# Tomiinek/Multilingual_Text_to_Speech

Measured on NVIDIA H100. Metric: mel-frames/sec (train fwd+bwd), higher is better.
Workload: dtype bf16

## Files before the change

### multilingual_text_to_speech_b200/csrc/decoder_persist_tc.cu

```cuda
#include <cuda.h>
#include <cuda_bf16.h>
#include "decoder_internal.cuh"
#include "tc_ptx.cuh"

namespace b200tts {

int tc_make_map3_bf16(void* map, const void* base, int d0, int d1, int d2, size_t stride1, size_t stride2, int b0, int b1, int b2);

namespace {

constexpr int NCW = 8;
constexpr int CT = 32 * NCW;
constexpr int PT = CT + 128;
constexpr int UNITS = 16;
constexpr int ROWS = 4 * UNITS;
constexpr int BT = 32;
constexpr int KB = 64;
constexpr int WTILE = ROWS * KB * 2;
constexpr int ATILE = BT * KB * 2;

struct TcLoopArgs {
    int B, T, D, K, Kp, RB, NBH;
    int nkb, nkb_h;
    int ch_h, n_h, ch_c, n_c, slot_kb;
    int alias_sum;
    int use_btab;
    const float* W; int ldw; int wcol_h, wcol_c;
    __nv_bfloat16* actb;
    float* actf; int ldf; int hcol;
    float* gates;
    float* cstate;
    const uint8_t* mask_h; const uint8_t* mask_c;
    int kind, training; float rate_h, rate_c;
    int L, M, A, KC;
    const float* Wq; float* qpart; float* qsave;
    const __nv_bfloat16* WcB;
    const __nv_bfloat16* memTf; int MT;
    const float* bias; const float* v;
    const uint4* memFf; int M16;
    const int* lengths;
    float* cum; float* align; long long align_bstride;
    unsigned* barrier; int* abort_flag;
    long long* prof;
    long long* prof2;
};

__device__ __forceinline__ uint32_t smem_u32(const void* p) { return (uint32_t)__cvta_generic_to_shared(p); }
__device__ __forceinline__ void mbar_init(uint64_t* bar, uint32_t count) {
    asm volatile("mbarrier.init.shared::cta.b64 [%0], %1;" ::"r"(smem_u32(bar)), "r"(count));
}
__device__ __forceinline__ void mbar_expect_tx(uint64_t* bar, uint32_t bytes) {
    asm volatile("mbarrier.arrive.expect_tx.shared::cta.b64 _, [%0], %1;" ::"r"(smem_u32(bar)), "r"(bytes) : "memory");
}
__device__ __forceinline__ void mbar_wait(uint64_t* bar, uint32_t parity) {
    const uint32_t addr = smem_u32(bar);
    const long long t0 = clock64();
    for (;;) {
        uint32_t done;
        asm volatile(
            "{\n\t.reg .pred p;\n\t"
            "mbarrier.try_wait.parity.shared::cta.b64 p, [%1], %2;\n\t"
            "selp.u32 %0, 1, 0, p;\n\t}"
            : "=r"(done)
            : "r"(addr), "r"(parity)
            : "memory");
        if (done) return;
        if (clock64() - t0 > 4000000000ll) __trap();
    }
}
__device__ __forceinline__ void tma_load_3d(void* smem, const CUtensorMap* map, uint64_t* bar, int c0, int c1, int c2) {
    asm volatile(
        "cp.async.bulk.tensor.3d.shared::cluster.global.mbarrier::complete_tx::bytes [%0], [%1, {%3, %4, %5}], [%2];"
        ::"r"(smem_u32(smem)), "l"(reinterpret_cast<uint64_t>(map)), "r"(smem_u32(bar)), "r"(c0), "r"(c1), "r"(c2)
        : "memory");
}
__device__ __forceinline__ void proxy_fence_global() { asm volatile("fence.proxy.async.global;" ::: "memory"); }
__device__ __forceinline__ void proxy_fence_shared() { asm volatile("fence.proxy.async.shared::cta;" ::: "memory"); }
__device__ __forceinline__ bool elect_one() {
    uint32_t pred;
    asm volatile("{\n\t.reg .pred P;\n\telect.sync _|P, 0xffffffff;\n\tselp.u32 %0, 1, 0, P;\n\t}" : "=r"(pred));
    return pred != 0;
}
__device__ __forceinline__ void l2_prefetch(const void* p) { asm volatile("prefetch.global.L2 [%0];" ::"l"(p)); }
__device__ __forceinline__ void cluster_arrive() { asm volatile("barrier.cluster.arrive.release.aligned;" ::: "memory"); }
__device__ __forceinline__ void cluster_wait() { asm volatile("barrier.cluster.wait.acquire.aligned;" ::: "memory"); }
__device__ __forceinline__ void st_peer_f32(const float* local_smem, uint32_t peer_rank, float v) {
    uint32_t ra;
    asm volatile("mapa.shared::cluster.u32 %0, %1, %2;" : "=r"(ra) : "r"(smem_u32(local_smem)), "r"(peer_rank));
    asm volatile("st.shared::cluster.f32 [%0], %1;" ::"r"(ra), "f"(v) : "memory");
}
__device__ __forceinline__ void st_async_peer_f32(const float* local_smem, const uint64_t* local_bar, uint32_t peer_rank, float v) {
    uint32_t ra, rb;
    asm volatile("mapa.shared::cluster.u32 %0, %1, %2;" : "=r"(ra) : "r"(smem_u32(local_smem)), "r"(peer_rank));
    asm volatile("mapa.shared::cluster.u32 %0, %1, %2;" : "=r"(rb) : "r"(smem_u32(local_bar)), "r"(peer_rank));
    asm volatile("st.async.shared::cluster.mbarrier::complete_tx::bytes.b32 [%0], %1, [%2];" ::"r"(ra), "r"(__float_as_uint(v)), "r"(rb) : "memory");
}
__device__ __forceinline__ void csync() { asm volatile("bar.sync 1, %0;" ::"n"(CT) : "memory"); }

__device__ __forceinline__ void ldmatrix_x4(uint32_t& r0, uint32_t& r1, uint32_t& r2, uint32_t& r3, const void* p) {
    const uint32_t addr = (uint32_t)__cvta_generic_to_shared(p);
    asm volatile("ldmatrix.sync.aligned.m8n8.x4.shared.b16 {%0,%1,%2,%3}, [%4];\n" : "=r"(r0), "=r"(r1), "=r"(r2), "=r"(r3) : "r"(addr));
}
__device__ __forceinline__ void mma_bf16(float (&c)[4], const uint32_t (&a)[4], uint32_t b0, uint32_t b1) {
    asm volatile("mma.sync.aligned.m16n8k16.row.col.f32.bf16.bf16.f32 {%0,%1,%2,%3}, {%4,%5,%6,%7}, {%8,%9}, {%0,%1,%2,%3};\n"
                 : "+f"(c[0]), "+f"(c[1]), "+f"(c[2]), "+f"(c[3])
                 : "r"(a[0]), "r"(a[1]), "r"(a[2]), "r"(a[3]), "r"(b0), "r"(b1));
}
__device__ __forceinline__ unsigned ld_acquire(const unsigned* p) {
    unsigned v;
    asm volatile("ld.acquire.gpu.global.u32 %0, [%1];\n" : "=r"(v) : "l"(p) : "memory");
    return v;
}
__device__ __forceinline__ uint32_t pack2(float lo, float hi) {
    __nv_bfloat162 v = __floats2bfloat162_rn(lo, hi);
    return *reinterpret_cast<uint32_t*>(&v);
}
__device__ __forceinline__ float tanh_fast(float x) {
    float y;
    asm("tanh.approx.f32 %0, %1;" : "=f"(y) : "f"(x));
    return y;
}

__device__ __forceinline__ float sigmoid_fast(float x) { return __fdividef(1.f, 1.f + __expf(-x)); }
__device__ __forceinline__ float tanh_exp(float x) { return 2.f * __fdividef(1.f, 1.f + __expf(-2.f * x)) - 1.f; }

__device__ __forceinline__ float cblock_max(float v, float* scratch) {
    const int lane = threadIdx.x & 31, warp = threadIdx.x >> 5;
    v = warp_max(v);
    csync();
    if (lane == 0) scratch[warp] = v;
    csync();
    float t = scratch[lane & (NCW - 1)];
#pragma unroll
    for (int o = NCW / 2; o > 0; o >>= 1) t = fmaxf(t, __shfl_xor_sync(0xffffffffu, t, o));
    return t;
}
__device__ __forceinline__ float cblock_sum(float v, float* scratch) {
    const int lane = threadIdx.x & 31, warp = threadIdx.x >> 5;
    v = warp_sum(v);
    csync();
    if (lane == 0) scratch[warp] = v;
    csync();
    float t = scratch[lane & (NCW - 1)];
#pragma unroll
    for (int o = NCW / 2; o > 0; o >>= 1) t += __shfl_xor_sync(0xffffffffu, t, o);
    return t;
}

struct NoOverlap { __device__ __forceinline__ void operator()() const {} };
template <typename Overlap = NoOverlap>
__device__ __forceinline__ bool grid_barrier(unsigned* counter, unsigned& target, unsigned nblocks, int* abort_flag, int* s_ok, Overlap overlap = Overlap()) {
    __syncthreads();
    if (threadIdx.x == 0) {
        target += nblocks;
        proxy_fence_global();
        asm volatile("red.release.gpu.global.add.u32 [%0], 1;" ::"l"(counter) : "memory");
    }
    overlap();
    if (threadIdx.x == 0) {
        int ok = 1;
        const long long t0 = clock64();
        unsigned polls = 0;
        for (;;) {
            unsigned v;
            asm volatile("ld.relaxed.gpu.global.u32 %0, [%1];" : "=r"(v) : "l"(counter) : "memory");
            if (v >= target) break;
            if ((++polls & 255u) == 0 && (clock64() - t0 > 4000000000ll || *reinterpret_cast<volatile int*>(abort_flag))) {
                ok = 0; *abort_flag = 1; break;
            }
        }
        asm volatile("fence.acquire.gpu;" ::: "memory");
        *s_ok = ok;
    }
    __syncthreads();
    return *s_ok != 0;
}

template <bool ATT, bool ALIAS>
__global__ void __launch_bounds__(PT, 1) lstm_loop_tc_kernel(const __grid_constant__ CUtensorMap tmH, const __grid_constant__ CUtensorMap tmC,
                                                             const TcLoopArgs p) {
    extern __shared__ __align__(1024) unsigned char smem_raw0[];
    unsigned char* smem_raw = reinterpret_cast<unsigned char*>((reinterpret_cast<uintptr_t>(smem_raw0) + 1023) & ~(uintptr_t)1023);
    __shared__ uint64_t full_bar, full2_bar, accum_bar, xchg_bar;
    __shared__ int s_ok;

    const int tid = threadIdx.x, lane = tid & 31;
    const int warp = __shfl_sync(0xffffffffu, tid >> 5, 0);
    const int cta = blockIdx.x;
    const int rb = cta % p.RB, bh = cta / p.RB;
    const int u0 = rb * UNITS, b0 = bh * BT;
    const int Kp = p.Kp, D = p.D, B = p.B;
    const unsigned nblocks = gridDim.x;
    unsigned* const bar_counter = p.barrier;
    const bool compute = warp < NCW;
    const bool is_mma = warp >= NCW;

    size_t off = 0;
    unsigned char* sW = smem_raw + off; off += (size_t)p.nkb * WTILE;
    unsigned char* ring = smem_raw + off;
    {
        const size_t ring_b = (size_t)p.slot_kb * ATILE, sum_b = (size_t)BT * (ROWS + 1) * 4;
        off += ALIAS ? (ring_b > sum_b ? ring_b : sum_b) : ring_b;
    }
    float* s_sum = ALIAS ? reinterpret_cast<float*>(ring) : reinterpret_cast<float*>(smem_raw + off);
    off += ALIAS ? 0 : (size_t)BT * (ROWS + 1) * 4;
    float* s_hs = reinterpret_cast<float*>(smem_raw + off); off += ATT ? (size_t)UNITS * (BT + 4) * 4 : 0;
    __nv_bfloat16* sWcB = reinterpret_cast<__nv_bfloat16*>(smem_raw + off); off += ATT ? (size_t)(p.A / 2) * 40 * 2 : 0;
    float* scratch = reinterpret_cast<float*>(smem_raw + off);

    for (int idx = tid; idx < ROWS * p.nkb * KB; idx += PT) {
        const int r = idx / (p.nkb * KB), k = idx % (p.nkb * KB);
        const int g = r / UNITS, u = r % UNITS;
        float w = 0.f;
        if (k < p.K && u0 + u < D) w = p.W[(size_t)(g * D + u0 + u) * p.ldw + (k < D ? p.wcol_h + k : p.wcol_c + (k - D))];
        const int kb = k / KB, kc = k % KB, chunk = kc >> 3, e = kc & 7;
        *reinterpret_cast<__nv_bfloat16*>(sW + (size_t)kb * WTILE + r * 128 + ((chunk ^ (r & 7)) << 4) + e * 2) = __float2bfloat16_rn(w);
    }
    if (ATT) {
        for (int idx = tid; idx < (p.A / 2) * 40; idx += PT) sWcB[idx] = p.WcB[(size_t)(cta & 1) * (p.A / 2) * 40 + idx];
    }
    if (tid == 0) {
        mbar_init(&full_bar, 1); mbar_init(&full2_bar, 1); mbar_init(&xchg_bar, 1);
        mbar_init(&accum_bar, 128);
        asm volatile("fence.mbarrier_init.release.cluster;" ::: "memory");
    }
    proxy_fence_shared();
    __syncthreads();
    if (ATT) { cluster_arrive(); cluster_wait(); }

    uint32_t mma_it = 0;
    long long rp[4] = {0, 0, 0, 0};
    float acc[16];
    auto mma_part = [&](int step, int part, bool signal_accum) {
        const long long t0 = clock64();
        long long t1 = t0;
        const int n = part ? p.n_h : (ALIAS ? p.n_c : 1), ch = part ? p.ch_h : p.ch_c;
        if (!ATT) {
            if (warp == NCW) {
                proxy_fence_global();
                if (elect_one()) {
                    for (int j = 0; j < n; ++j) {
                        uint64_t* fb = j ? &full2_bar : &full_bar;
                        mbar_expect_tx(fb, (uint32_t)ch * ATILE);
                        tma_load_3d(ring + (size_t)j * ch * ATILE, &tmH, fb, 0, step * B + b0, j * ch);
                    }
                }
                __syncwarp();
            }
            for (int j = 0; j < n; ++j) {
                mbar_wait(j ? &full2_bar : &full_bar, mma_it & 1);
                if (j == 0) t1 = clock64();
                tcx::wgmma_fence();
                for (int c = 0; c < ch; ++c) {
                    const uint64_t adesc = tcx::make_sw128_desc(smem_u32(sW + (size_t)(j * ch + c) * WTILE));
                    const uint64_t bdesc = tcx::make_sw128_desc(smem_u32(ring + (size_t)(j * ch + c) * ATILE));
#pragma unroll
                    for (int k = 0; k < KB / 16; ++k) tcx::wgmma_m64n32<0, 0>(acc, adesc + 2 * k, bdesc + 2 * k, (j | c | k) != 0);
                }
                tcx::wgmma_commit();
            }
            ++mma_it;
            tcx::wgmma_wait<0>();
            tcx::wgmma_fence_acc(acc);
        } else {
            for (int j = 0; j < n; ++j) {
                if (warp == NCW) {
                    if (j == 0) proxy_fence_global();
                    if (elect_one()) {
                        if (ALIAS) proxy_fence_shared();
                        mbar_expect_tx(&full_bar, (uint32_t)ch * ATILE);
                        tma_load_3d(ring, part ? &tmH : &tmC, &full_bar, 0, step * B + b0, part ? j * ch : p.nkb_h + j * ch);
                    }
                    __syncwarp();
                }
                mbar_wait(&full_bar, mma_it & 1);
                ++mma_it;
                if (j == 0) t1 = clock64();
                const int kb0 = part ? j * ch : p.nkb_h + j * ch;
                tcx::wgmma_fence();
                for (int c = 0; c < ch; ++c) {
                    const uint64_t adesc = tcx::make_sw128_desc(smem_u32(sW + (size_t)(kb0 + c) * WTILE));
                    const uint64_t bdesc = tcx::make_sw128_desc(smem_u32(ring + (size_t)c * ATILE));
#pragma unroll
                    for (int k = 0; k < KB / 16; ++k)
                        tcx::wgmma_m64n32<0, 0>(acc, adesc + 2 * k, bdesc + 2 * k, (part == 1 && j == 0 && c == 0 && k == 0) ? 0u : 1u);
                }
                tcx::wgmma_commit();
                tcx::wgmma_wait<0>();
                tcx::wgmma_fence_acc(acc);
                tcx::wg_sync(NCW / 4);
            }
        }
        if (signal_accum) {
            const int row = 16 * (warp - NCW) + (lane >> 2), col = 2 * (lane & 3);
#pragma unroll
            for (int r = 0; r < 16; ++r) s_sum[(8 * (r >> 2) + col + (r & 1)) * (ROWS + 1) + row + 8 * ((r >> 1) & 1)] = acc[r];
            tcx::mbar_arrive(&accum_bar);
        }
        rp[2 * part] += t1 - t0; rp[2 * part + 1] += clock64() - t1;
    };

    uint32_t wqh[2][2] = {{0u, 0u}, {0u, 0u}}, wql[2][2] = {{0u, 0u}, {0u, 0u}};
    if (ATT && compute) {
        const int g = lane >> 2, tq = lane & 3;
#pragma unroll
        for (int j = 0; j < 2; ++j)
#pragma unroll
            for (int r2 = 0; r2 < 2; ++r2) {
                const int a = (2 * warp + j) * 8 + g, u = u0 + 2 * tq + 8 * r2;
                const float x0 = (a < p.A && u < D) ? p.Wq[(size_t)a * D + u] : 0.f, x1 = (a < p.A && u + 1 < D) ? p.Wq[(size_t)a * D + u + 1] : 0.f;
                const __nv_bfloat16 h0 = __float2bfloat16_rn(x0), h1 = __float2bfloat16_rn(x1);
                __nv_bfloat162 hp2; hp2.x = h0; hp2.y = h1;
                wqh[j][r2] = *reinterpret_cast<uint32_t*>(&hp2);
                wql[j][r2] = pack2(x0 - __bfloat162float(h0), x1 - __bfloat162float(h1));
            }
    }
    const float inv_h = 1.f / (1.f - p.rate_h), inv_c = 1.f / (1.f - p.rate_c);
    unsigned target = 0;
    long long prof_acc[8] = {0, 0, 0, 0, 0, 0, 0, 0};
    long long prof_t = clock64();
#define PROF_MARK(slot)                                                      \
    do {                                                                     \
        if (p.prof && tid == 0) { const long long now = clock64(); prof_acc[slot] += now - prof_t; prof_t = now; } \
    } while (0)

    if (is_mma) mma_part(0, 1, !ATT || p.nkb_h == p.nkb);

    float pre[2][6];
    uint8_t pm[2][2];
    auto prefetch = [&](int step, bool state) {
#pragma unroll
        for (int e2 = 0; e2 < 2; ++e2) {
            const int idx = tid + e2 * CT;
            const int bl = idx / UNITS, uu = idx % UNITS, b = b0 + bl, u = u0 + uu;
            pm[e2][0] = 1; pm[e2][1] = 1;
#pragma unroll
            for (int j = 0; j < 4; ++j) pre[e2][j] = 0.f;
            if (state) { pre[e2][4] = 0.f; pre[e2][5] = 0.f; }
            if (b < B && u < D) {
                const size_t g0 = ((size_t)step * B + b) * 4 * D + u, mi = ((size_t)step * B + b) * D + u;
                pre[e2][0] = p.gates[g0]; pre[e2][1] = p.gates[g0 + D]; pre[e2][2] = p.gates[g0 + 2 * D]; pre[e2][3] = p.gates[g0 + 3 * D];
                if (state) {
                    pre[e2][4] = p.cstate[mi];
                    pre[e2][5] = p.actf[((size_t)step * B + b) * p.ldf + p.hcol + u];
                }
                if (p.training && p.mask_h) pm[e2][0] = p.mask_h[mi];
                if (p.training && p.mask_c) pm[e2][1] = p.mask_c[mi];
            }
        }
    };
    auto prefetch_l2 = [&](int step) {
        if (step >= p.T) return;
#pragma unroll
        for (int e2 = 0; e2 < 2; ++e2) {
            const int idx = tid + e2 * CT;
            const int bl = idx / UNITS, uu = idx % UNITS, b = b0 + bl, u = u0 + uu;
            if (b < B && u < D && (uu & 7) == 0) {
                const size_t g0 = ((size_t)step * B + b) * 4 * D + u, mi = ((size_t)step * B + b) * D + u;
                l2_prefetch(p.gates + g0); l2_prefetch(p.gates + g0 + D); l2_prefetch(p.gates + g0 + 2 * D); l2_prefetch(p.gates + g0 + 3 * D);
                if (uu == 0 && p.training && p.mask_h) l2_prefetch(p.mask_h + mi);
                if (uu == 0 && p.training && p.mask_c) l2_prefetch(p.mask_c + mi);
            }
        }
    };
    if (compute) { prefetch_l2(0); prefetch(0, true); prefetch_l2(1); }

    int att_len = 0;
    if (ATT && (cta >> 1) < B) { const int l0 = p.lengths[cta >> 1]; att_len = l0 < 0 ? 0 : (l0 > p.L ? p.L : l0); }
    bool alive = true;
    for (int i = 0; i < p.T && alive; ++i) {
        if (ATT && p.nkb_h < p.nkb && is_mma) mma_part(i, 0, true);
        if (compute) {
            mbar_wait(&accum_bar, i & 1);
            PROF_MARK(0);
#pragma unroll
            for (int e2 = 0; e2 < 2; ++e2) {
                const int idx = tid + e2 * CT;
                const int bl = idx / UNITS, uu = idx % UNITS, b = b0 + bl, u = u0 + uu;
                float hs = 0.f;
                if (b < B && u < D) {
                    const size_t g0 = ((size_t)i * B + b) * 4 * D + u;
                    const float zi = pre[e2][0] + s_sum[bl * (ROWS + 1) + uu];
                    const float zf = pre[e2][1] + s_sum[bl * (ROWS + 1) + UNITS + uu];
                    const float zg = pre[e2][2] + s_sum[bl * (ROWS + 1) + 2 * UNITS + uu];
                    const float zo = pre[e2][3] + s_sum[bl * (ROWS + 1) + 3 * UNITS + uu];
                    const float gi = sigmoid_fast(zi), gf = sigmoid_fast(zf), gg = tanh_exp(zg), go = sigmoid_fast(zo);
                    const size_t bu = (size_t)b * D + u;
                    const float cp = pre[e2][4];
                    float cn = gf * cp + gi * gg;
                    float hn = go * tanh_exp(cn);
                    p.gates[g0] = gi; p.gates[g0 + D] = gf; p.gates[g0 + 2 * D] = gg; p.gates[g0 + 3 * D] = go;
                    if (p.kind == B200TTS_CELL_ZONEOUT) {
                        const float hp = pre[e2][5];
                        if (p.training) {
                            float dh = hn - hp, dc = cn - cp;
                            if (p.mask_h) dh = dh * (float)pm[e2][0] * inv_h;
                            if (p.mask_c) dc = dc * (float)pm[e2][1] * inv_c;
                            hn = (1.f - p.rate_h) * dh + hp;
                            cn = (1.f - p.rate_c) * dc + cp;
                        } else {
                            hn = p.rate_h * hp + (1.f - p.rate_h) * hn;
                            cn = p.rate_c * cp + (1.f - p.rate_c) * cn;
                        }
                    } else if (p.training && p.mask_h) {
                        hn = hn * (float)pm[e2][0] * inv_h;
                    }
                    p.cstate[(size_t)(i + 1) * B * D + bu] = cn;
                    p.actf[((size_t)(i + 1) * B + b) * p.ldf + p.hcol + u] = hn;
                    p.actb[((size_t)(i + 1) * B + b) * Kp + u] = __float2bfloat16_rn(hn);
                    hs = hn;
                    pre[e2][4] = cn; pre[e2][5] = hn;
                }
                if (ATT) s_hs[uu * (BT + 4) + bl] = hs;
            }
            if (ATT) {
                csync();
                {
                    const int g = lane >> 2, tq = lane & 3;
                    uint32_t ah[2][4], al[2][4];
#pragma unroll
                    for (int mt = 0; mt < 2; ++mt)
#pragma unroll
                        for (int r4 = 0; r4 < 4; ++r4) {
                            const int bl = mt * 16 + g + 8 * (r4 & 1), k = 2 * tq + 8 * (r4 >> 1);
                            const float x0 = s_hs[k * (BT + 4) + bl], x1 = s_hs[(k + 1) * (BT + 4) + bl];
                            const __nv_bfloat16 h0 = __float2bfloat16_rn(x0), h1 = __float2bfloat16_rn(x1);
                            __nv_bfloat162 hp2; hp2.x = h0; hp2.y = h1;
                            ah[mt][r4] = *reinterpret_cast<uint32_t*>(&hp2);
                            al[mt][r4] = pack2(x0 - __bfloat162float(h0), x1 - __bfloat162float(h1));
                        }
#pragma unroll
                    for (int mt = 0; mt < 2; ++mt)
#pragma unroll
                        for (int j = 0; j < 2; ++j) {
                            float acc[4] = {0.f, 0.f, 0.f, 0.f};
                            mma_bf16(acc, ah[mt], wqh[j][0], wqh[j][1]);
                            mma_bf16(acc, al[mt], wqh[j][0], wqh[j][1]);
                            mma_bf16(acc, ah[mt], wql[j][0], wql[j][1]);
                            const int a = (2 * warp + j) * 8 + 2 * tq;
                            const int bA = b0 + mt * 16 + g, bB = bA + 8;
                            if (bA < B) *reinterpret_cast<float2*>(p.qpart + ((size_t)rb * B + bA) * p.A + a) = make_float2(acc[0], acc[1]);
                            if (bB < B) *reinterpret_cast<float2*>(p.qpart + ((size_t)rb * B + bB) * p.A + a) = make_float2(acc[2], acc[3]);
                        }
                }
            }
        }
        PROF_MARK(1);
        if (ALIAS) proxy_fence_shared();
        if (!grid_barrier(bar_counter, target, nblocks, p.abort_flag, &s_ok)) { alive = false; break; }
        PROF_MARK(2);

        if (i + 1 < p.T) {
            if (is_mma) mma_part(i + 1, 1, !ATT || p.nkb_h == p.nkb);
            if (compute) { prefetch_l2(i + 2); if (!ATT) prefetch(i + 1, false); }
        }

        if (ATT) {
            const int pc = cta >> 1, hf = cta & 1;
            if (compute && pc < B) {
                const int b = pc, L = p.L, A = p.A, AH = p.A / 2, M = p.M, half = (p.KC - 1) / 2, L16 = p.MT * 16;
                float* qb = scratch;
                float* vv = qb + AH;
                float* bias_s = vv + AH;
                float* cum_s = bias_s + AH;
                float* e = cum_s + L16;
                float* eq = e + L16;
                float* epart = eq + 2 * L16;
                float* red = epart + 2 * L16;
                float* cred = red + 64;
                uint32_t* Ph = reinterpret_cast<uint32_t*>(cred + 16 * AH);
                uint32_t* Pl = Ph + (L16 + 48);
                uint2* btab = reinterpret_cast<uint2*>(Pl + (L16 + 48));
                const int len = att_len;
                const int mtiles = (len + 15) / 16, ktiles = mtiles;
                if (i == 0) {
                    for (int a2 = tid; a2 < AH; a2 += CT) { vv[a2] = p.v[hf * AH + a2]; bias_s[a2] = p.bias[hf * AH + a2]; }
                    for (int l = tid; l < L16; l += CT) cum_s[l] = l < L ? p.cum[(size_t)b * L + l] : 0.f;
                    csync();
                }
                constexpr int KTMAX = 12;
                const int mt_lo = hf * ((p.M16 + 1) / 2), mt_hi = min(p.M16, mt_lo + (p.M16 + 1) / 2);
                uint4 nraw[2];
                uint4 av[KTMAX];
                {
                    const int a4 = tid & 15, sl = tid >> 4;
                    const int per = (p.RB + 15) / 16, r0 = sl * per, r1 = min(p.RB, r0 + per);
                    float4 qv[4];
#pragma unroll
                    for (int j = 0; j < 4; ++j)
                        qv[j] = (r0 + j < r1) ? __ldcg(reinterpret_cast<const float4*>(p.qpart + ((size_t)(r0 + j) * B + b) * A + hf * AH) + a4)
                                              : make_float4(0.f, 0.f, 0.f, 0.f);
                    if (warp < 2 * mtiles) {
                        const uint4* mf = reinterpret_cast<const uint4*>(p.memTf + (((size_t)b * p.MT + (warp >> 1)) * 32 + lane) * 64) + hf * 4 + (warp & 1) * 2;
                        nraw[0] = __ldg(mf); nraw[1] = __ldg(mf + 1);
                    }
                    if (mt_lo + warp < mt_hi) {
                        const uint4* fr = p.memFf + (((size_t)b * p.M16 + mt_lo + warp) * p.MT) * 32 + lane;
#pragma unroll
                        for (int j = 0; j < KTMAX; ++j)
                            if (j < ktiles) av[j] = __ldg(fr + (size_t)j * 32);
                    }
                    for (int x = tid; x < L16 + 48; x += CT) {
                        float c0 = 0.f, c1 = 0.f;
                        const int la = x - half, lb = x + 1 - half;
                        if (la >= 0 && la < L) c0 = cum_s[la];
                        if (lb >= 0 && lb < L) c1 = cum_s[lb];
                        const __nv_bfloat16 h0 = __float2bfloat16_rn(c0), h1 = __float2bfloat16_rn(c1);
                        __nv_bfloat162 hp2; hp2.x = h0; hp2.y = h1;
                        Ph[x] = *reinterpret_cast<uint32_t*>(&hp2);
                        Pl[x] = pack2(c0 - __bfloat162float(h0), c1 - __bfloat162float(h1));
                    }
                    float4 qs = make_float4(0.f, 0.f, 0.f, 0.f);
#pragma unroll
                    for (int j = 0; j < 4; ++j) { qs.x += qv[j].x; qs.y += qv[j].y; qs.z += qv[j].z; qs.w += qv[j].w; }
                    for (int r = r0 + 4; r < r1; r += 4) {
#pragma unroll
                        for (int j = 0; j < 4; ++j)
                            if (r + j < r1) {
                                const float4 v4 = __ldcg(reinterpret_cast<const float4*>(p.qpart + ((size_t)(r + j) * B + b) * A + hf * AH) + a4);
                                qs.x += v4.x; qs.y += v4.y; qs.z += v4.z; qs.w += v4.w;
                            }
                    }
                    *reinterpret_cast<float4*>(cred + sl * AH + a4 * 4) = qs;
                    csync();
                    for (int a2 = tid; a2 < AH; a2 += CT) {
                        float q = 0.f;
#pragma unroll
                        for (int sl2 = 0; sl2 < 16; ++sl2) q += cred[sl2 * AH + a2];
                        p.qsave[((size_t)i * B + b) * A + hf * AH + a2] = q;
                        qb[a2] = q + bias_s[a2];
                    }
                }
                csync();
                PROF_MARK(3);
                {
                    const int g = lane >> 2, tq = lane & 3;
                    for (int job = warp; job < 2 * mtiles; job += NCW) {
                        const int mt = job >> 1, qh = job & 1, l0 = mt * 16;
                        const uint4 raw[2] = {nraw[0], nraw[1]};
                        if (job + NCW < 2 * mtiles) {
                            const int nj = job + NCW;
                            const uint4* mf = reinterpret_cast<const uint4*>(p.memTf + (((size_t)b * p.MT + (nj >> 1)) * 32 + lane) * 64) + hf * 4 + (nj & 1) * 2;
                            nraw[0] = __ldg(mf); nraw[1] = __ldg(mf + 1);
                        }
                        float sacc[4][4];
#pragma unroll
                        for (int nt = 0; nt < 4; ++nt)
#pragma unroll
                            for (int e4 = 0; e4 < 4; ++e4) sacc[nt][e4] = 0.f;
#pragma unroll
                        for (int ks = 0; ks < 2; ++ks) {
                            const int x = l0 + ks * 16 + g + 2 * tq;
                            const uint32_t ah[4] = {Ph[x], Ph[x + 8], Ph[x + 8], Ph[x + 16]};
                            const uint32_t al[4] = {Pl[x], Pl[x + 8], Pl[x + 8], Pl[x + 16]};
#pragma unroll
                            for (int np = 0; np < 2; ++np) {
                                uint32_t bfr[4];
                                ldmatrix_x4(bfr[0], bfr[1], bfr[2], bfr[3],
                                            sWcB + (size_t)((qh * 2 + np) * 16 + (lane & 7) + ((lane >> 4) << 3)) * 40 + ks * 16 + ((lane >> 3) & 1) * 8);
                                mma_bf16(sacc[2 * np], ah, bfr[0], bfr[1]);
                                mma_bf16(sacc[2 * np], al, bfr[0], bfr[1]);
                                mma_bf16(sacc[2 * np + 1], ah, bfr[2], bfr[3]);
                                mma_bf16(sacc[2 * np + 1], al, bfr[2], bfr[3]);
                            }
                        }
                        float e0 = 0.f, e1 = 0.f;
#pragma unroll
                        for (int c4 = 0; c4 < 2; ++c4) {
                            const uint32_t words[4] = {raw[c4].x, raw[c4].y, raw[c4].z, raw[c4].w};
#pragma unroll
                            for (int h2 = 0; h2 < 2; ++h2) {
                                const int nt = 2 * c4 + h2, a0 = (qh * 4 + nt) * 8 + 2 * tq;
                                const float2 m01 = __bfloat1622float2(*reinterpret_cast<const __nv_bfloat162*>(&words[2 * h2]));
                                const float2 m23 = __bfloat1622float2(*reinterpret_cast<const __nv_bfloat162*>(&words[2 * h2 + 1]));
                                e0 = fmaf(vv[a0], tanh_fast(sacc[nt][0] + qb[a0] + m01.x), e0);
                                e0 = fmaf(vv[a0 + 1], tanh_fast(sacc[nt][1] + qb[a0 + 1] + m01.y), e0);
                                e1 = fmaf(vv[a0], tanh_fast(sacc[nt][2] + qb[a0] + m23.x), e1);
                                e1 = fmaf(vv[a0 + 1], tanh_fast(sacc[nt][3] + qb[a0 + 1] + m23.y), e1);
                            }
                        }
                        e0 += __shfl_xor_sync(0xffffffffu, e0, 1); e0 += __shfl_xor_sync(0xffffffffu, e0, 2);
                        e1 += __shfl_xor_sync(0xffffffffu, e1, 1); e1 += __shfl_xor_sync(0xffffffffu, e1, 2);
                        if (tq == 0) { eq[qh * L16 + l0 + g] = e0; eq[qh * L16 + l0 + g + 8] = e1; }
                    }
                }
                csync();
                if (tid == 0) mbar_expect_tx(&xchg_bar, (uint32_t)L16 * 4);
                for (int l = tid; l < L16; l += CT) {
                    const float v = l < mtiles * 16 ? eq[l] + eq[L16 + l] : 0.f;
                    epart[hf * L16 + l] = v;
                    st_async_peer_f32(epart + hf * L16 + l, &xchg_bar, (uint32_t)(hf ^ 1), v);
                }
                csync();
                mbar_wait(&xchg_bar, i & 1);
                PROF_MARK(4);
                float mx = -INFINITY;
                for (int l = tid; l < len; l += CT) { const float ev = epart[l] + epart[L16 + l]; e[l] = ev; mx = fmaxf(mx, ev); }
                mx = cblock_max(mx, red);
                float sum = 0.f;
                for (int l = tid; l < len; l += CT) { const float ex = expf(e[l] - mx); e[l] = ex; sum += ex; }
                sum = cblock_sum(sum, red + 32);
                float* cum_next = p.cum + ((size_t)(i + 1) * B + b) * L;
                const float inv_sum = 1.f / sum;
                for (int l = tid; l < L16; l += CT) {
                    const float w = l < len ? e[l] * inv_sum : 0.f;
                    e[l] = w;
                    if (l < L) {
                        const float cn = cum_s[l] + w;
                        cum_s[l] = cn;
                        if (hf == 0) p.align[(size_t)b * p.align_bstride + (size_t)i * L + l] = w;
                        else cum_next[l] = cn;
                    }
                }
                csync();
                if (p.use_btab) {
                    for (int idx = tid; idx < ktiles * 32; idx += CT) {
                        const int kt = idx >> 5, gg = (idx >> 2) & 7, tt = idx & 3;
                        uint2 f = make_uint2(0u, 0u);
                        if (gg < 2) {
                            const float* wl = e + kt * 16 + 2 * tt;
                            const float w0 = wl[0], w1 = wl[1], w2 = wl[8], w3 = wl[9];
                            const float h0 = __bfloat162float(__float2bfloat16_rn(w0)), h1 = __bfloat162float(__float2bfloat16_rn(w1));
                            const float h2 = __bfloat162float(__float2bfloat16_rn(w2)), h3 = __bfloat162float(__float2bfloat16_rn(w3));
                            f = gg == 0 ? make_uint2(pack2(h0, h1), pack2(h2, h3)) : make_uint2(pack2(w0 - h0, w1 - h1), pack2(w2 - h2, w3 - h3));
                        }
                        btab[idx] = f;
                    }
                    csync();
                }
                PROF_MARK(5);
                {
                    const int g = lane >> 2, tq = lane & 3;
                    uint32_t bfr[KTMAX][2];
                    auto build_b = [&](int kt0) {
                        if (p.use_btab) {
#pragma unroll
                            for (int j = 0; j < KTMAX; ++j) {
                                bfr[j][0] = 0u; bfr[j][1] = 0u;
                                if (kt0 + j < ktiles) { const uint2 f = btab[(kt0 + j) * 32 + lane]; bfr[j][0] = f.x; bfr[j][1] = f.y; }
                            }
                            return;
                        }
#pragma unroll
                        for (int j = 0; j < KTMAX; ++j) {
                            bfr[j][0] = 0u; bfr[j][1] = 0u;
                            if (kt0 + j < ktiles) {
                                const float* wl = e + (kt0 + j) * 16 + 2 * tq;
                                const float w0 = wl[0], w1 = wl[1], w2 = wl[8], w3 = wl[9];
                                const float h0 = __bfloat162float(__float2bfloat16_rn(w0)), h1 = __bfloat162float(__float2bfloat16_rn(w1));
                                const float h2 = __bfloat162float(__float2bfloat16_rn(w2)), h3 = __bfloat162float(__float2bfloat16_rn(w3));
                                const float s0 = g == 0 ? h0 : (g == 1 ? w0 - h0 : 0.f), s1 = g == 0 ? h1 : (g == 1 ? w1 - h1 : 0.f);
                                const float s2 = g == 0 ? h2 : (g == 1 ? w2 - h2 : 0.f), s3 = g == 0 ? h3 : (g == 1 ? w3 - h3 : 0.f);
                                bfr[j][0] = pack2(s0, s1); bfr[j][1] = pack2(s2, s3);
                            }
                        }
                    };
                    const bool single = ktiles <= KTMAX;
                    if (single) build_b(0);
                    for (int mt = mt_lo + warp; mt < mt_hi; mt += NCW) {
                        float dacc[4] = {0.f, 0.f, 0.f, 0.f}, dacc2[4] = {0.f, 0.f, 0.f, 0.f};
                        for (int kt0 = 0; kt0 < ktiles; kt0 += KTMAX) {
                            if (kt0 > 0 || mt != mt_lo + warp) {
                                const uint4* fr = p.memFf + (((size_t)b * p.M16 + mt) * p.MT) * 32 + lane;
#pragma unroll
                                for (int j = 0; j < KTMAX; ++j)
                                    if (kt0 + j < ktiles) av[j] = __ldg(fr + (size_t)(kt0 + j) * 32);
                            }
                            if (!single) build_b(kt0);
#pragma unroll
                            for (int j = 0; j < KTMAX; j += 2) {
                                if (kt0 + j < ktiles) {
                                    const uint32_t af[4] = {av[j].x, av[j].y, av[j].z, av[j].w};
                                    mma_bf16(dacc, af, bfr[j][0], bfr[j][1]);
                                }
                                if (kt0 + j + 1 < ktiles) {
                                    const uint32_t af[4] = {av[j + 1].x, av[j + 1].y, av[j + 1].z, av[j + 1].w};
                                    mma_bf16(dacc2, af, bfr[j + 1][0], bfr[j + 1][1]);
                                }
                            }
                        }
                        if (tq == 0) {
                            const int m0 = mt * 16 + g;
                            const float c0 = (dacc[0] + dacc2[0]) + (dacc[1] + dacc2[1]), c1 = (dacc[2] + dacc2[2]) + (dacc[3] + dacc2[3]);
                            if (m0 < M) {
                                p.actf[((size_t)(i + 1) * B + b) * p.ldf + m0] = c0;
                                p.actb[((size_t)(i + 1) * B + b) * Kp + D + m0] = __float2bfloat16_rn(c0);
                            }
                            if (m0 + 8 < M) {
                                p.actf[((size_t)(i + 1) * B + b) * p.ldf + m0 + 8] = c1;
                                p.actb[((size_t)(i + 1) * B + b) * Kp + D + m0 + 8] = __float2bfloat16_rn(c1);
                            }
                        }
                    }
                }
            }
            PROF_MARK(6);
            if (!grid_barrier(bar_counter, target, nblocks, p.abort_flag, &s_ok, [&]() { if (compute && i + 1 < p.T) prefetch(i + 1, false); })) {
                alive = false; break;
            }
            PROF_MARK(7);
        }
    }
    if (p.prof && tid == 0)
        for (int k = 0; k < 8; ++k) p.prof[(size_t)cta * 8 + k] = prof_acc[k];
#undef PROF_MARK
    if (p.prof2 && warp == NCW && lane == 0)
        for (int k = 0; k < 4; ++k) p.prof2[(size_t)cta * 8 + k] = rp[k];
}

size_t tc_loop_smem_bytes(int nkb, int slot_kb, int A, bool att, int L, bool alias = false) {
    const size_t ring_b = (size_t)slot_kb * ATILE, sum_b = (size_t)BT * (ROWS + 1) * 4;
    size_t b = 1024 + (size_t)nkb * WTILE + (alias ? (ring_b > sum_b ? ring_b : sum_b) : ring_b + sum_b);
    if (att) {
        const int L16 = (L + 15) / 16 * 16;
        b += (size_t)UNITS * (BT + 4) * 4 + (size_t)(A / 2) * 40 * 2;
        b += ((size_t)3 * (A / 2) + 6 * L16 + 64 + 16 * (A / 2) + 2 * (L16 + 48)) * 4;
    }
    return b;
}
constexpr size_t SMEM_LIMIT = 227 * 1024 - 1088;

int pick_slot(int nkb, int A, bool att, int L, int want, bool alias = false) {
    int kb = want;
    while (kb >= 1 && tc_loop_smem_bytes(nkb, kb, A, att, L, alias) > SMEM_LIMIT) --kb;
    return kb;
}
int largest_divisor_le(int n, int cap) {
    for (int d = cap < n ? cap : n; d >= 1; --d)
        if (n % d == 0) return d;
    return 1;
}

}

TcPersistGeom tc_persist_geom(const b200tts_decoder_shape& s) {
    TcPersistGeom g{};
    g.nkb_att = (s.D + s.M + KB - 1) / KB;
    g.nkb_gen = (s.D + KB - 1) / KB;
    g.nkb_h = s.D / KB;
    g.Kp_att = g.nkb_att * KB;
    g.Kp_gen = g.nkb_gen * KB;
    const int nkb_c = g.nkb_att - g.nkb_h;
    g.alias_att = 0;
    g.slot_att = pick_slot(g.nkb_att, s.A, true, s.L, g.nkb_h);
    if (g.slot_att < nkb_c) {
        g.alias_att = 1;
        g.slot_att = pick_slot(g.nkb_att, s.A, true, s.L, g.nkb_h, true);
    }
    g.ch_c_att = g.slot_att >= 1 ? largest_divisor_le(nkb_c, g.slot_att) : 0;
    g.n_c_att = g.ch_c_att >= 1 ? nkb_c / g.ch_c_att : 0;
    g.ch_h_att = g.slot_att >= 1 ? largest_divisor_le(g.nkb_h, g.slot_att) : 0;
    g.slot_gen = pick_slot(g.nkb_gen, s.A, false, 0, g.nkb_gen);
    g.ch_h_gen = g.slot_gen >= 1 ? largest_divisor_le(g.nkb_gen, g.slot_gen) : 0;
    if (g.slot_gen >= g.nkb_gen && g.nkb_gen % 2 == 0) g.ch_h_gen = g.nkb_gen / 2;
    return g;
}

bool tc_persist_supported(const b200tts_decoder_shape& s) {
    if (s.D % KB != 0 || s.D % UNITS != 0) return false;
    const int RB = s.D / UNITS, NBH = (s.B + BT - 1) / BT;
    if (RB * NBH > NUM_SMS || s.B > RB * NBH) return false;
    if (s.K > 32 || s.A != 128) return false;
    const TcPersistGeom g = tc_persist_geom(s);
    return g.ch_c_att >= 1 && g.ch_c_att <= 256 && g.slot_att >= g.ch_c_att && g.ch_h_att >= 1 && g.ch_h_gen >= 1 && g.slot_att >= 2 &&
           g.slot_gen >= g.nkb_gen;
}

static int launch_tc_loop(bool att, const TcLoopArgs& a, const CUtensorMap& tmH, const CUtensorMap& tmC, size_t smem, cudaStream_t st) {
    void* fn = att ? (a.alias_sum ? (void*)lstm_loop_tc_kernel<true, true> : (void*)lstm_loop_tc_kernel<true, false>) : (void*)lstm_loop_tc_kernel<false, false>;
    B200_CUDA(cudaFuncSetAttribute(fn, cudaFuncAttributeMaxDynamicSharedMemorySize, (int)smem));
    const int grid = a.RB * a.NBH;
    TcLoopArgs args = a;
    CUtensorMap mapH = tmH, mapC = tmC;
    void* params[] = {&mapH, &mapC, &args};
    cudaLaunchConfig_t cfg{};
    cfg.gridDim = dim3(grid); cfg.blockDim = dim3(PT); cfg.dynamicSmemBytes = smem; cfg.stream = st;
    cudaLaunchAttribute attrs[2];
    attrs[0].id = cudaLaunchAttributeCooperative;
    attrs[0].val.cooperative = 1;
    cfg.attrs = attrs; cfg.numAttrs = 1;
    if (att) {
        B200_REQUIRE(grid % 2 == 0 && grid / 2 >= a.B, "wgmma attention loop: %d CTAs cannot form %d pairs", grid, a.B);
        attrs[1].id = cudaLaunchAttributeClusterDimension;
        attrs[1].val.clusterDim.x = 2; attrs[1].val.clusterDim.y = 1; attrs[1].val.clusterDim.z = 1;
        cfg.numAttrs = 2;
        int nclusters = 0;
        B200_CUDA(cudaOccupancyMaxActiveClusters(&nclusters, fn, &cfg));
        B200_REQUIRE(nclusters * 2 >= grid, "wgmma attention loop: only %d CTA pairs can be co-resident, %d needed", nclusters, grid / 2);
    } else {
        int per_sm = 0, dev = 0, sms = 0;
        B200_CUDA(cudaOccupancyMaxActiveBlocksPerMultiprocessor(&per_sm, fn, PT, smem));
        B200_CUDA(cudaGetDevice(&dev));
        B200_CUDA(cudaDeviceGetAttribute(&sms, cudaDevAttrMultiProcessorCount, dev));
        B200_REQUIRE(per_sm * sms >= grid, "wgmma persistent loop: %d CTAs cannot be co-resident (%d per SM x %d SMs)", grid, per_sm, sms);
    }
    KernelTimer kt(att ? "lstm_loop_tc_kernel<att>" : "lstm_loop_tc_kernel<gen>", st);
    B200_CUDA(cudaLaunchKernelExC(&cfg, fn, params));
    B200_LAUNCH_CHECK();
    return B200TTS_OK;
}

int tc_persist_att_loop(const b200tts_decoder_shape& s, const b200tts_decoder_params& w, const b200tts_decoder_inputs& in,
                        const DecoderLayout& fl, float* ws, unsigned char* pws, float* align, cudaStream_t st) {
    const PersistLayout l = persist_layout(s);
    const TcPersistGeom g = tc_persist_geom(s);
    const int B = s.B, T = s.T, D = s.D, M = s.M, MD = M + D;
    __nv_bfloat16* aib = reinterpret_cast<__nv_bfloat16*>(pws + l.aib);
    unsigned* barrier = reinterpret_cast<unsigned*>(pws + l.barrier);
    B200_CUDA(cudaMemsetAsync(aib, 0, (size_t)(g.Kp_att != MD ? (size_t)(T + 1) : 1) * B * g.Kp_att * 2, st));
    B200_CUDA(cudaMemsetAsync(barrier, 0, 256, st));
    CUtensorMap tmH, tmC;
    B200_TRY(tc_make_map3_bf16(&tmH, aib, KB, (T + 1) * B, g.nkb_att, (size_t)g.Kp_att * 2, 128, KB, BT, g.ch_h_att));
    B200_TRY(tc_make_map3_bf16(&tmC, aib, KB, (T + 1) * B, g.nkb_att, (size_t)g.Kp_att * 2, 128, KB, BT, g.ch_c_att));
    TcLoopArgs a{};
    a.B = B; a.T = T; a.D = D; a.K = MD; a.Kp = g.Kp_att; a.RB = D / UNITS; a.NBH = (B + BT - 1) / BT;
    a.nkb = g.nkb_att; a.nkb_h = g.nkb_h; a.ch_h = g.ch_h_att; a.n_h = g.nkb_h / g.ch_h_att; a.ch_c = g.ch_c_att; a.n_c = g.n_c_att;
    a.alias_sum = g.alias_att;
    a.slot_kb = g.ch_h_att > g.ch_c_att ? g.ch_h_att : g.ch_c_att;
    a.W = ws + fl.wcat_att; a.ldw = MD; a.wcol_h = M; a.wcol_c = 0;
    a.actb = aib; a.actf = ws + fl.ai; a.ldf = MD; a.hcol = M;
    a.gates = ws + fl.ga; a.cstate = ws + fl.ca;
    a.mask_h = in.mask_att_h; a.mask_c = in.mask_att_c; a.kind = s.cell_kind; a.training = s.training; a.rate_h = s.rate_h; a.rate_c = s.rate_c;
    a.L = s.L; a.M = M; a.A = s.A; a.KC = s.K;
    a.Wq = w.attn_query; a.qpart = ws + fl.qpart; a.qsave = ws + fl.q;
    a.WcB = reinterpret_cast<const __nv_bfloat16*>(pws + l.wcb);
    a.memTf = reinterpret_cast<const __nv_bfloat16*>(pws + l.memTf); a.MT = l.MT;
    a.bias = w.attn_bias; a.v = w.attn_energy;
    a.memFf = reinterpret_cast<const uint4*>(pws + l.memFf); a.M16 = l.M16;
    a.lengths = in.text_lengths; a.cum = ws + fl.cum;
    a.align = align; a.align_bstride = (long long)T * s.L;
    a.barrier = barrier; a.abort_flag = reinterpret_cast<int*>(barrier + 32);
    a.prof = reinterpret_cast<long long*>(pws + l.barrier + 256);
    a.prof2 = a.prof + 2 * NUM_SMS * 8;
    size_t smem = tc_loop_smem_bytes(g.nkb_att, a.slot_kb, s.A, true, s.L, g.alias_att != 0);
    const size_t tab = (size_t)l.MT * 32 * 8;
    a.use_btab = smem + tab <= SMEM_LIMIT ? 1 : 0;
    if (a.use_btab) smem += tab;
    return launch_tc_loop(true, a, tmH, tmC, smem, st);
}

int tc_persist_gen_loop(const b200tts_decoder_shape& s, const b200tts_decoder_params& w, const b200tts_decoder_inputs& in,
                        const DecoderLayout& fl, float* ws, unsigned char* pws, cudaStream_t st) {
    const PersistLayout l = persist_layout(s);
    const TcPersistGeom g = tc_persist_geom(s);
    const int B = s.B, T = s.T, D = s.D;
    __nv_bfloat16* hgb = reinterpret_cast<__nv_bfloat16*>(pws + l.hgb);
    unsigned* barrier = reinterpret_cast<unsigned*>(pws + l.barrier);
    B200_CUDA(cudaMemsetAsync(hgb, 0, (size_t)(g.Kp_gen != D ? (size_t)(T + 1) : 1) * B * g.Kp_gen * 2, st));
    B200_CUDA(cudaMemsetAsync(barrier, 0, 256, st));
    CUtensorMap tmH;
    B200_TRY(tc_make_map3_bf16(&tmH, hgb, KB, (T + 1) * B, g.nkb_gen, (size_t)g.Kp_gen * 2, 128, KB, BT, g.ch_h_gen));
    TcLoopArgs a{};
    a.B = B; a.T = T; a.D = D; a.K = D; a.Kp = g.Kp_gen; a.RB = D / UNITS; a.NBH = (B + BT - 1) / BT;
    a.nkb = g.nkb_gen; a.nkb_h = g.nkb_gen; a.ch_h = g.ch_h_gen; a.n_h = g.nkb_gen / g.ch_h_gen; a.ch_c = 0; a.n_c = 0; a.alias_sum = 0; a.use_btab = 0; a.slot_kb = g.nkb_gen;
    a.W = w.gen_w_hh; a.ldw = D; a.wcol_h = 0; a.wcol_c = 0;
    a.actb = hgb; a.actf = ws + fl.hg; a.ldf = D; a.hcol = 0;
    a.gates = ws + fl.gg; a.cstate = ws + fl.cg;
    a.mask_h = in.mask_gen_h; a.mask_c = in.mask_gen_c; a.kind = s.cell_kind; a.training = s.training; a.rate_h = s.rate_h; a.rate_c = s.rate_c;
    a.barrier = barrier; a.abort_flag = reinterpret_cast<int*>(barrier + 32);
    a.prof = reinterpret_cast<long long*>(pws + l.barrier + 256) + NUM_SMS * 8;
    a.prof2 = a.prof + 2 * NUM_SMS * 8;
    return launch_tc_loop(false, a, tmH, tmH, tc_loop_smem_bytes(g.nkb_gen, a.slot_kb, s.A, false, 0), st);
}

}
```

Before: 677,700.

## Specialize MMA and compute warps with setmaxnreg register rebalancing

Splits the persistent LSTM kernel into two warp roles with separate control flow. The MMA producer warps run their own loop, mirroring the grid barrier with paired __syncthreads and exit early, after lowering their register budget with setmaxnreg.dec. The compute warps raise their budget with setmaxnreg.inc so the gate and attention code has more registers and spills less. The trap path moves into a noinline function, and the profiling accumulators move to shared memory in the attention variant to save registers. The main risk is barrier-count mismatch between the two roles, which could deadlock or mis-synchronise.

New measurement: 743,600, median of 6. +9.7%, better.

```diff
diff --git a/multilingual_text_to_speech_b200/csrc/decoder_persist_tc.cu b/multilingual_text_to_speech_b200/csrc/decoder_persist_tc.cu
--- a/multilingual_text_to_speech_b200/csrc/decoder_persist_tc.cu
+++ b/multilingual_text_to_speech_b200/csrc/decoder_persist_tc.cu
@@ -12,6 +12,9 @@
 constexpr int NCW = 8;
 constexpr int CT = 32 * NCW;
 constexpr int PT = CT + 128;
+constexpr int R_MMA = 56;
+constexpr int R_CMP = 224;
+static_assert(128 * R_MMA + CT * R_CMP <= PT * 168 && R_MMA % 8 == 0 && R_CMP % 8 == 0, "register split exceeds the CTA's allocation");
 constexpr int UNITS = 16;
 constexpr int ROWS = 4 * UNITS;
 constexpr int BT = 32;
@@ -52,6 +55,7 @@
 __device__ __forceinline__ void mbar_expect_tx(uint64_t* bar, uint32_t bytes) {
     asm volatile("mbarrier.arrive.expect_tx.shared::cta.b64 _, [%0], %1;" ::"r"(smem_u32(bar)), "r"(bytes) : "memory");
 }
+__device__ __noinline__ __attribute__((noreturn)) void watchdog_trap() { __trap(); }
 __device__ __forceinline__ void mbar_wait(uint64_t* bar, uint32_t parity) {
     const uint32_t addr = smem_u32(bar);
     const long long t0 = clock64();
@@ -65,7 +69,7 @@
             : "r"(addr), "r"(parity)
             : "memory");
         if (done) return;
-        if (clock64() - t0 > 4000000000ll) __trap();
+        if (clock64() - t0 > 4000000000ll) watchdog_trap();
     }
 }
 __device__ __forceinline__ void tma_load_3d(void* smem, const CUtensorMap* map, uint64_t* bar, int c0, int c1, int c2) {
@@ -96,6 +100,10 @@
     asm volatile("st.async.shared::cluster.mbarrier::complete_tx::bytes.b32 [%0], %1, [%2];" ::"r"(ra), "r"(__float_as_uint(v)), "r"(rb) : "memory");
 }
 __device__ __forceinline__ void csync() { asm volatile("bar.sync 1, %0;" ::"n"(CT) : "memory"); }
+template <int N>
+__device__ __forceinline__ void setmaxnreg_dec() { asm volatile("setmaxnreg.dec.sync.aligned.u32 %0;" ::"n"(N)); }
+template <int N>
+__device__ __forceinline__ void setmaxnreg_inc() { asm volatile("setmaxnreg.inc.sync.aligned.u32 %0;" ::"n"(N)); }
 
 __device__ __forceinline__ void ldmatrix_x4(uint32_t& r0, uint32_t& r1, uint32_t& r2, uint32_t& r3, const void* p) {
     const uint32_t addr = (uint32_t)__cvta_generic_to_shared(p);
@@ -175,6 +183,11 @@
     __syncthreads();
     return *s_ok != 0;
 }
+__device__ __forceinline__ bool grid_barrier_mma(const int* s_ok) {
+    __syncthreads();
+    __syncthreads();
+    return *s_ok != 0;
+}
 
 template <bool ATT, bool ALIAS>
 __global__ void __launch_bounds__(PT, 1) lstm_loop_tc_kernel(const __grid_constant__ CUtensorMap tmH, const __grid_constant__ CUtensorMap tmC,
@@ -192,7 +205,6 @@
     const int Kp = p.Kp, D = p.D, B = p.B;
     const unsigned nblocks = gridDim.x;
     unsigned* const bar_counter = p.barrier;
-    const bool compute = warp < NCW;
     const bool is_mma = warp >= NCW;
 
     size_t off = 0;
@@ -300,8 +312,24 @@
         rp[2 * part] += t1 - t0; rp[2 * part + 1] += clock64() - t1;
     };
 
+    if (is_mma) {
+        setmaxnreg_dec<R_MMA>();
+        mma_part(0, 1, !ATT || p.nkb_h == p.nkb);
+        for (int i = 0; i < p.T; ++i) {
+            if (ATT && p.nkb_h < p.nkb) mma_part(i, 0, true);
+            if (ALIAS) proxy_fence_shared();
+            if (!grid_barrier_mma(&s_ok)) break;
+            if (i + 1 < p.T) mma_part(i + 1, 1, !ATT || p.nkb_h == p.nkb);
+            if (ATT && !grid_barrier_mma(&s_ok)) break;
+        }
+        if (p.prof2 && warp == NCW && lane == 0)
+            for (int k = 0; k < 4; ++k) p.prof2[(size_t)cta * 8 + k] = rp[k];
+        return;
+    }
+    setmaxnreg_inc<R_CMP>();
+
     uint32_t wqh[2][2] = {{0u, 0u}, {0u, 0u}}, wql[2][2] = {{0u, 0u}, {0u, 0u}};
-    if (ATT && compute) {
+    if (ATT) {
         const int g = lane >> 2, tq = lane & 3;
 #pragma unroll
         for (int j = 0; j < 2; ++j)
@@ -317,14 +345,18 @@
     }
     const float inv_h = 1.f / (1.f - p.rate_h), inv_c = 1.f / (1.f - p.rate_c);
     unsigned target = 0;
-    long long prof_acc[8] = {0, 0, 0, 0, 0, 0, 0, 0};
-    long long prof_t = clock64();
+    __shared__ long long prof_sm[9];
+    long long prof_rg[9];
+    long long* const prof_acc = ATT ? prof_sm : prof_rg;
+    if (tid == 0) {
+        for (int k = 0; k < 8; ++k) prof_acc[k] = 0;
+        prof_acc[8] = clock64();
+    }
 #define PROF_MARK(slot)                                                      \
     do {                                                                     \
-        if (p.prof && tid == 0) { const long long now = clock64(); prof_acc[slot] += now - prof_t; prof_t = now; } \
+        if (p.prof && tid == 0) { const long long now = clock64(); prof_acc[slot] += now - prof_acc[8]; prof_acc[8] = now; } \
     } while (0)
 
-    if (is_mma) mma_part(0, 1, !ATT || p.nkb_h == p.nkb);
 
     float pre[2][6];
     uint8_t pm[2][2];
@@ -363,86 +395,83 @@
             }
         }
     };
-    if (compute) { prefetch_l2(0); prefetch(0, true); prefetch_l2(1); }
+    prefetch_l2(0); prefetch(0, true); prefetch_l2(1);
 
     int att_len = 0;
     if (ATT && (cta >> 1) < B) { const int l0 = p.lengths[cta >> 1]; att_len = l0 < 0 ? 0 : (l0 > p.L ? p.L : l0); }
     bool alive = true;
     for (int i = 0; i < p.T && alive; ++i) {
-        if (ATT && p.nkb_h < p.nkb && is_mma) mma_part(i, 0, true);
-        if (compute) {
-            mbar_wait(&accum_bar, i & 1);
-            PROF_MARK(0);
-#pragma unroll
-            for (int e2 = 0; e2 < 2; ++e2) {
-                const int idx = tid + e2 * CT;
-                const int bl = idx / UNITS, uu = idx % UNITS, b = b0 + bl, u = u0 + uu;
-                float hs = 0.f;
-                if (b < B && u < D) {
-                    const size_t g0 = ((size_t)i * B + b) * 4 * D + u;
-                    const float zi = pre[e2][0] + s_sum[bl * (ROWS + 1) + uu];
-                    const float zf = pre[e2][1] + s_sum[bl * (ROWS + 1) + UNITS + uu];
-                    const float zg = pre[e2][2] + s_sum[bl * (ROWS + 1) + 2 * UNITS + uu];
-                    const float zo = pre[e2][3] + s_sum[bl * (ROWS + 1) + 3 * UNITS + uu];
-                    const float gi = sigmoid_fast(zi), gf = sigmoid_fast(zf), gg = tanh_exp(zg), go = sigmoid_fast(zo);
-                    const size_t bu = (size_t)b * D + u;
-                    const float cp = pre[e2][4];
-                    float cn = gf * cp + gi * gg;
-                    float hn = go * tanh_exp(cn);
-                    p.gates[g0] = gi; p.gates[g0 + D] = gf; p.gates[g0 + 2 * D] = gg; p.gates[g0 + 3 * D] = go;
-                    if (p.kind == B200TTS_CELL_ZONEOUT) {
-                        const float hp = pre[e2][5];
-                        if (p.training) {
-                            float dh = hn - hp, dc = cn - cp;
-                            if (p.mask_h) dh = dh * (float)pm[e2][0] * inv_h;
-                            if (p.mask_c) dc = dc * (float)pm[e2][1] * inv_c;
-                            hn = (1.f - p.rate_h) * dh + hp;
-                            cn = (1.f - p.rate_c) * dc + cp;
-                        } else {
-                            hn = p.rate_h * hp + (1.f - p.rate_h) * hn;
-                            cn = p.rate_c * cp + (1.f - p.rate_c) * cn;
-                        }
-                    } else if (p.training && p.mask_h) {
-                        hn = hn * (float)pm[e2][0] * inv_h;
-                    }
-                    p.cstate[(size_t)(i + 1) * B * D + bu] = cn;
-                    p.actf[((size_t)(i + 1) * B + b) * p.ldf + p.hcol + u] = hn;
-                    p.actb[((size_t)(i + 1) * B + b) * Kp + u] = __float2bfloat16_rn(hn);
-                    hs = hn;
-                    pre[e2][4] = cn; pre[e2][5] = hn;
-                }
-                if (ATT) s_hs[uu * (BT + 4) + bl] = hs;
-            }
-            if (ATT) {
-                csync();
-                {
-                    const int g = lane >> 2, tq = lane & 3;
-                    uint32_t ah[2][4], al[2][4];
-#pragma unroll
-                    for (int mt = 0; mt < 2; ++mt)
-#pragma unroll
-                        for (int r4 = 0; r4 < 4; ++r4) {
-                            const int bl = mt * 16 + g + 8 * (r4 & 1), k = 2 * tq + 8 * (r4 >> 1);
-                            const float x0 = s_hs[k * (BT + 4) + bl], x1 = s_hs[(k + 1) * (BT + 4) + bl];
-                            const __nv_bfloat16 h0 = __float2bfloat16_rn(x0), h1 = __float2bfloat16_rn(x1);
-                            __nv_bfloat162 hp2; hp2.x = h0; hp2.y = h1;
-                            ah[mt][r4] = *reinterpret_cast<uint32_t*>(&hp2);
-                            al[mt][r4] = pack2(x0 - __bfloat162float(h0), x1 - __bfloat162float(h1));
-                        }
-#pragma unroll
-                    for (int mt = 0; mt < 2; ++mt)
-#pragma unroll
-                        for (int j = 0; j < 2; ++j) {
-                            float acc[4] = {0.f, 0.f, 0.f, 0.f};
-                            mma_bf16(acc, ah[mt], wqh[j][0], wqh[j][1]);
-                            mma_bf16(acc, al[mt], wqh[j][0], wqh[j][1]);
-                            mma_bf16(acc, ah[mt], wql[j][0], wql[j][1]);
-                            const int a = (2 * warp + j) * 8 + 2 * tq;
-                            const int bA = b0 + mt * 16 + g, bB = bA + 8;
-                            if (bA < B) *reinterpret_cast<float2*>(p.qpart + ((size_t)rb * B + bA) * p.A + a) = make_float2(acc[0], acc[1]);
-                            if (bB < B) *reinterpret_cast<float2*>(p.qpart + ((size_t)rb * B + bB) * p.A + a) = make_float2(acc[2], acc[3]);
-                        }
-                }
+        mbar_wait(&accum_bar, i & 1);
+        PROF_MARK(0);
+#pragma unroll
+        for (int e2 = 0; e2 < 2; ++e2) {
+            const int idx = tid + e2 * CT;
+            const int bl = idx / UNITS, uu = idx % UNITS, b = b0 + bl, u = u0 + uu;
+            float hs = 0.f;
+            if (b < B && u < D) {
+                const size_t g0 = ((size_t)i * B + b) * 4 * D + u;
+                const float zi = pre[e2][0] + s_sum[bl * (ROWS + 1) + uu];
+                const float zf = pre[e2][1] + s_sum[bl * (ROWS + 1) + UNITS + uu];
+                const float zg = pre[e2][2] + s_sum[bl * (ROWS + 1) + 2 * UNITS + uu];
+                const float zo = pre[e2][3] + s_sum[bl * (ROWS + 1) + 3 * UNITS + uu];
+                const float gi = sigmoid_fast(zi), gf = sigmoid_fast(zf), gg = tanh_exp(zg), go = sigmoid_fast(zo);
+                const size_t bu = (size_t)b * D + u;
+                const float cp = pre[e2][4];
+                float cn = gf * cp + gi * gg;
+                float hn = go * tanh_exp(cn);
+                p.gates[g0] = gi; p.gates[g0 + D] = gf; p.gates[g0 + 2 * D] = gg; p.gates[g0 + 3 * D] = go;
+                if (p.kind == B200TTS_CELL_ZONEOUT) {
+                    const float hp = pre[e2][5];
+                    if (p.training) {
+                        float dh = hn - hp, dc = cn - cp;
+                        if (p.mask_h) dh = dh * (float)pm[e2][0] * inv_h;
+                        if (p.mask_c) dc = dc * (float)pm[e2][1] * inv_c;
+                        hn = (1.f - p.rate_h) * dh + hp;
+                        cn = (1.f - p.rate_c) * dc + cp;
+                    } else {
+                        hn = p.rate_h * hp + (1.f - p.rate_h) * hn;
+                        cn = p.rate_c * cp + (1.f - p.rate_c) * cn;
+                    }
+                } else if (p.training && p.mask_h) {
+                    hn = hn * (float)pm[e2][0] * inv_h;
+                }
+                p.cstate[(size_t)(i + 1) * B * D + bu] = cn;
+                p.actf[((size_t)(i + 1) * B + b) * p.ldf + p.hcol + u] = hn;
+                p.actb[((size_t)(i + 1) * B + b) * Kp + u] = __float2bfloat16_rn(hn);
+                hs = hn;
+                pre[e2][4] = cn; pre[e2][5] = hn;
+            }
+            if (ATT) s_hs[uu * (BT + 4) + bl] = hs;
+        }
+        if (ATT) {
+            csync();
+            {
+                const int g = lane >> 2, tq = lane & 3;
+                uint32_t ah[2][4], al[2][4];
+#pragma unroll
+                for (int mt = 0; mt < 2; ++mt)
+#pragma unroll
+                    for (int r4 = 0; r4 < 4; ++r4) {
+                        const int bl = mt * 16 + g + 8 * (r4 & 1), k = 2 * tq + 8 * (r4 >> 1);
+                        const float x0 = s_hs[k * (BT + 4) + bl], x1 = s_hs[(k + 1) * (BT + 4) + bl];
+                        const __nv_bfloat16 h0 = __float2bfloat16_rn(x0), h1 = __float2bfloat16_rn(x1);
+                        __nv_bfloat162 hp2; hp2.x = h0; hp2.y = h1;
+                        ah[mt][r4] = *reinterpret_cast<uint32_t*>(&hp2);
+                        al[mt][r4] = pack2(x0 - __bfloat162float(h0), x1 - __bfloat162float(h1));
+                    }
+#pragma unroll
+                for (int mt = 0; mt < 2; ++mt)
+#pragma unroll
+                    for (int j = 0; j < 2; ++j) {
+                        float acc[4] = {0.f, 0.f, 0.f, 0.f};
+                        mma_bf16(acc, ah[mt], wqh[j][0], wqh[j][1]);
+                        mma_bf16(acc, al[mt], wqh[j][0], wqh[j][1]);
+                        mma_bf16(acc, ah[mt], wql[j][0], wql[j][1]);
+                        const int a = (2 * warp + j) * 8 + 2 * tq;
+                        const int bA = b0 + mt * 16 + g, bB = bA + 8;
+                        if (bA < B) *reinterpret_cast<float2*>(p.qpart + ((size_t)rb * B + bA) * p.A + a) = make_float2(acc[0], acc[1]);
+                        if (bB < B) *reinterpret_cast<float2*>(p.qpart + ((size_t)rb * B + bB) * p.A + a) = make_float2(acc[2], acc[3]);
+                    }
             }
         }
         PROF_MARK(1);
@@ -450,14 +479,11 @@
         if (!grid_barrier(bar_counter, target, nblocks, p.abort_flag, &s_ok)) { alive = false; break; }
         PROF_MARK(2);
 
-        if (i + 1 < p.T) {
-            if (is_mma) mma_part(i + 1, 1, !ATT || p.nkb_h == p.nkb);
-            if (compute) { prefetch_l2(i + 2); if (!ATT) prefetch(i + 1, false); }
-        }
+        if (i + 1 < p.T) { prefetch_l2(i + 2); if (!ATT) prefetch(i + 1, false); }
 
         if (ATT) {
             const int pc = cta >> 1, hf = cta & 1;
-            if (compute && pc < B) {
+            if (pc < B) {
                 const int b = pc, L = p.L, A = p.A, AH = p.A / 2, M = p.M, half = (p.KC - 1) / 2, L16 = p.MT * 16;
                 float* qb = scratch;
                 float* vv = qb + AH;
@@ -695,7 +721,7 @@
                 }
             }
             PROF_MARK(6);
-            if (!grid_barrier(bar_counter, target, nblocks, p.abort_flag, &s_ok, [&]() { if (compute && i + 1 < p.T) prefetch(i + 1, false); })) {
+            if (!grid_barrier(bar_counter, target, nblocks, p.abort_flag, &s_ok, [&]() { if (i + 1 < p.T) prefetch(i + 1, false); })) {
                 alive = false; break;
             }
             PROF_MARK(7);
@@ -704,8 +730,6 @@
     if (p.prof && tid == 0)
         for (int k = 0; k < 8; ++k) p.prof[(size_t)cta * 8 + k] = prof_acc[k];
 #undef PROF_MARK
-    if (p.prof2 && warp == NCW && lane == 0)
-        for (int k = 0; k < 4; ++k) p.prof2[(size_t)cta * 8 + k] = rp[k];
 }
 
 size_t tc_loop_smem_bytes(int nkb, int slot_kb, int A, bool att, int L, bool alias = false) {
```
